# NickB42/mri-image-generation

Hardware: NVIDIA B200
Metric: volumes/sec (3D LDM DDPM sampling) (higher is better)
Workload: dtype bf16

## Files before the change

mri_image_generation_b200/csrc/gemm_tc.cu:

```cuda
#include <cuda.h>
#include <cuda_bf16.h>
#include <cuda_runtime.h>
#include <stdlib.h>
#include <string.h>

#include "../../include/mri_b200.h"
#include "common.h"
#include "ptx.cuh"

#ifdef MRI_GEMM_FINE_TRACE
#define FT_START() do { if (trace != nullptr) ft_t = clock64(); } while (0)
#define FT_ADD(k) do { if (trace != nullptr) { const long long n_ = clock64(); ft[k] += (unsigned long long)(n_ - ft_t); ft_t = n_; } } while (0)
#else
#define FT_START() do { } while (0)
#define FT_ADD(k) do { } while (0)
#endif

namespace mri {

constexpr int kBlockM = 128;
constexpr int kBlockK = 64;
constexpr int kUmmaK = 16;
constexpr int kSlabBytes = kBlockM * 128;
#ifndef MRI_EPI_WARPS
#define MRI_EPI_WARPS 4
#endif
constexpr int kEpiWarps = MRI_EPI_WARPS;
static_assert(kEpiWarps == 4 || kEpiWarps == 8, "one or two epilogue warps per TMEM lane quadrant");
constexpr int kSplit = kEpiWarps / 4;
constexpr int kEpiWarp0 = kEpiWarps == 8 ? 4 : 2;
constexpr int kThreads = (kEpiWarp0 + kEpiWarps) * 32;
constexpr int kEpiThreads = kEpiWarps * 32;
constexpr int kRegsProducer = 104, kRegsEpilogue = 200;
constexpr int kMaxStages = 8;
constexpr int kChunkBytes = kBlockM * 128;
constexpr int kStagingBytes = 2 * kChunkBytes;
constexpr int kPartialLd = 256;
constexpr int kMaxStatGroups = 32;
constexpr int kSmemLimit = 227 * 1024;
constexpr int kXTileBytes = 2 * 160 * 128;
constexpr int kXYTileBytes = 2 * 180 * 128;
constexpr int kXStages = 3;

__host__ __device__ inline int stage_bytes(int block_n, int swap_ab) {
  return swap_ab ? 3 * kSlabBytes : kSlabBytes + block_n * 128;
}

struct Work {
  int cls, n0, nbox;
  int tix[2][4], org[2][4];
};

struct Geom {
  int boxes_per_class;
  int groups_per_class;
  long long n_tiles;
  float rcp_ntn, rcp_gpc, rcp_te[4];
  int te[4], od[4];
};

__device__ __forceinline__ void fdivmod(int n, int d, float rcp, int& q, int& r) {
  q = __float2int_rz(__int2float_rn(n) * rcp);
  r = n - q * d;
  if (r < 0) {
    --q;
    r += d;
  } else if (r >= d) {
    ++q;
    r -= d;
  }
}

__device__ __forceinline__ Geom make_geom(const MriGemmArgs& p) {
  Geom g;
  g.boxes_per_class = p.tiles[0] * p.tiles[1] * p.tiles[2] * p.tiles[3];
  g.groups_per_class = p.swap_ab ? (g.boxes_per_class + 1) / 2 : g.boxes_per_class;
  g.n_tiles = (long long)p.n_tiles_n * p.n_class * g.groups_per_class;
  g.rcp_ntn = 1.0f / (float)p.n_tiles_n;
  g.rcp_gpc = 1.0f / (float)g.groups_per_class;
  const int f = p.tile_fast_dim;
#pragma unroll
  for (int k = 0; k < 4; ++k) {
    g.od[k] = (f == 0) ? k : (k == 0 ? f : (k <= f ? k - 1 : k));
    g.te[k] = g.od[k] == 0 ? p.tiles[0] : (g.od[k] == 1 ? p.tiles[1] : (g.od[k] == 2 ? p.tiles[2] : p.tiles[3]));
    g.rcp_te[k] = 1.0f / (float)g.te[k];
  }
  return g;
}

__device__ __forceinline__ int pick4(const int (&a)[4], int i) {
  return i == 0 ? a[0] : (i == 1 ? a[1] : (i == 2 ? a[2] : a[3]));
}

__device__ __forceinline__ void decode_tile(const MriGemmArgs& p, const Geom& g, int tile, Work& w) {
  int nt, pr;
  fdivmod(tile, p.n_tiles_n, g.rcp_ntn, pr, nt);
  int rem;
  fdivmod(pr, g.groups_per_class, g.rcp_gpc, w.cls, rem);
  w.n0 = nt * p.block_n;
  int b0 = rem;
  w.nbox = 1;
  if (p.swap_ab) {
    b0 = 2 * rem;
    w.nbox = (b0 + 1 < g.boxes_per_class) ? 2 : 1;
  }
#pragma unroll
  for (int h = 0; h < 2; ++h) {
    int b = b0 + h;
    int v[4];
#pragma unroll
    for (int k = 0; k < 4; ++k) {
      int qn;
      fdivmod(b, g.te[k], g.rcp_te[k], qn, v[k]);
      b = qn;
    }
#pragma unroll
    for (int i = 0; i < 4; ++i) {
      w.tix[h][i] = g.od[0] == i ? v[0] : (g.od[1] == i ? v[1] : (g.od[2] == i ? v[2] : v[3]));
      w.org[h][i] = w.tix[h][i] * p.box[i];
    }
  }
}

struct Sched {
  int n_kb, G, GA, q;
  long long rem_units;
  long long n_tiles, rem;
};

__device__ __forceinline__ Sched make_sched(const MriGemmArgs& p, long long n_tiles, int G) {
  Sched s;
  s.n_kb = p.n_kb;
  s.G = G;
  s.n_tiles = n_tiles;
  if (p.sched == 0) {
    s.q = 0;
    s.rem = 0;
    s.rem_units = 0;
    s.GA = 0;
  } else {
    s.q = (int)(n_tiles / G);
    s.rem = n_tiles - (long long)s.q * G;
    s.rem_units = s.rem * p.n_kb;
    const int min_share = (p.n_kb + 3) / 4 > 8 ? (p.n_kb + 3) / 4 : 8;
    const long long ga = s.rem_units / min_share;
    s.GA = (int)(ga < 1 ? (s.rem > 0 ? 1 : 0) : (ga > G ? G : ga));
  }
  return s;
}

__device__ __forceinline__ void range_a(const Sched& s, int r, long long& u0, long long& u1) {
  if (r >= s.GA) {
    u0 = u1 = s.rem_units;
    return;
  }
  u0 = s.rem_units * r / s.GA;
  u1 = s.rem_units * (r + 1) / s.GA;
}

struct SegIter {
  long long u, u1;
  long long tb, tb1;
  int n_kb;
  __device__ __forceinline__ void init(const MriGemmArgs& p, const Sched& s, int r) {
    n_kb = s.n_kb;
    if (p.sched == 0) {
      u = u1 = 0;
      tb = s.n_tiles * r / s.G;
      tb1 = s.n_tiles * (r + 1) / s.G;
    } else {
      range_a(s, r, u, u1);
      tb = s.rem + (long long)r * s.q;
      tb1 = tb + s.q;
    }
  }
  __device__ __forceinline__ bool next(int& tile, int& kb0, int& len, long long& seg_end) {
    if (u < u1) {
      tile = (int)(u / n_kb);
      kb0 = (int)(u - (long long)tile * n_kb);
      const long long left = u1 - u;
      len = (int)(left < (long long)(n_kb - kb0) ? left : (long long)(n_kb - kb0));
      u += len;
      seg_end = u;
      return true;
    }
    if (tb < tb1) {
      tile = (int)tb++;
      kb0 = 0;
      len = n_kb;
      seg_end = -1;
      return true;
    }
    return false;
  }
};

__device__ __forceinline__ uint32_t ld_acquire_gpu(const int32_t* p) {
  uint32_t v;
  asm volatile("ld.acquire.gpu.global.u32 %0, [%1];" : "=r"(v) : "l"(p) : "memory");
  return v;
}
__device__ __forceinline__ void st_release_gpu(int32_t* p, uint32_t v) {
  asm volatile("st.release.gpu.global.u32 [%0], %1;" ::"l"(p), "r"(v) : "memory");
}

__device__ __forceinline__ int count_contributors(const Sched& s, int my_r, long long pos,
                                                  long long tile_end) {
  int n = 0;
  int rr = my_r + 1;
  while (pos < tile_end) {
    long long a, b;
    range_a(s, rr, a, b);
    pos = b < tile_end ? b : tile_end;
    ++rr;
    ++n;
  }
  return n;
}

__device__ __forceinline__ void wait_contributors(const MriGemmArgs& p, int first_cta, int n) {
  for (int j = 0; j < n; ++j) {
    const int32_t* f = p.sk_flags + (first_cta - j);
    const uint64_t t0 = globaltimer_ns();
    while (ld_acquire_gpu(f) == 0u) {
      if (globaltimer_ns() - t0 > 4000000000ull) {
        printf("mri_b200: stream-K partial wait timeout (block %d waits for %d)\n",
               (int)blockIdx.x, first_cta - j);
        __trap();
      }
    }
  }
}

__device__ __forceinline__ float4* partial_ptr(const MriGemmArgs& p, int cta, int lane128, int col) {
  return reinterpret_cast<float4*>(p.sk_partials) +
         ((size_t)cta * (kPartialLd / 4) + (size_t)(col >> 2)) * kBlockM + lane128;
}

__global__ void __launch_bounds__(kThreads, 1)
gemm_tc_kernel(const __grid_constant__ MriGemmArgs p) {
  extern __shared__ uint8_t smem_raw[];
  __shared__ __align__(8) uint64_t bars[2 * kMaxStages + 5 + kXStages];
  __shared__ uint32_t tmem_holder;
  __shared__ double s_stats[kMaxStatGroups * 2];
  __shared__ int s_pos_info[kBlockM];
  __shared__ uint32_t s_vmask[4];
  __shared__ uint32_t s_winfo[kMaxStages];

  const int warp = uniform((int)(threadIdx.x >> 5));
  const int lane = threadIdx.x & 31;

  const uint32_t smem_base = (smem_u32(smem_raw) + 1023u) & ~1023u;
  const int S = p.stages;
  const int block_n = p.block_n;
  const bool swap = p.swap_ab != 0;
  const int sbytes = stage_bytes(block_n, p.swap_ab);
  const uint32_t stag = smem_base + (uint32_t)(p.xreuse ? S * kSlabBytes + (p.xreuse == 2 ? 2 * kXYTileBytes : ((p.staging2 || p.stages > 4) ? 2 : kXStages) * kXTileBytes)
                                                        : S * sbytes);
  const uint32_t bar0 = smem_u32(bars);
  auto full_bar = [&](int s) { return bar0 + 8u * s; };
  auto empty_bar = [&](int s) { return bar0 + 8u * (kMaxStages + s); };
  auto tmem_full_bar = [&](int b) { return bar0 + 8u * (2 * kMaxStages + b); };
  auto tmem_empty_bar = [&](int b) { return bar0 + 8u * (2 * kMaxStages + 2 + b); };
  const uint32_t resid_bar = bar0 + 8u * (2 * kMaxStages + 4);
  auto xempty_bar = [&](int s) { return bar0 + 8u * (2 * kMaxStages + 5 + s); };
  const bool xreuse = p.xreuse != 0;
  const bool xy = p.xreuse == 2;
  const int XS = (xy || p.staging2 || p.stages > 4) ? 2 : kXStages;
  const uint32_t x_tile_bytes = xy ? (uint32_t)kXYTileBytes : (uint32_t)kXTileBytes;
  const int x_box_rows = xy ? 180 : 160;
  const uint32_t x_ring = smem_base + (uint32_t)(S * kSlabBytes);

  const int n_kb = p.n_kb;
  const int G = (int)gridDim.x;
  const int my_r = G - 1 - (int)blockIdx.x;
  __shared__ Geom s_geom;
  __shared__ Sched s_sch;
  if (threadIdx.x == 0) {
    s_geom = make_geom(p);
    s_sch = make_sched(p, s_geom.n_tiles, G);
  }
  const Geom& geom = s_geom;
  const Sched& sch = s_sch;
  const int rows_in_box = p.box[0] * p.box[1] * p.box[2] * p.box[3];
  const bool dual = !swap && block_n <= 128;

  if (warp == 0 && lane == 0) {
    for (int s = 0; s < S; ++s) {
      mbar_init(full_bar(s), 1);
      mbar_init(empty_bar(s), 1);
    }
    for (int b = 0; b < 2; ++b) {
      mbar_init(tmem_full_bar(b), 1);
      mbar_init(tmem_empty_bar(b), kEpiThreads / 32);
    }
    mbar_init(resid_bar, 1);
    for (int xs = 0; xs < kXStages; ++xs) mbar_init(xempty_bar(xs), 1);
// ... 780 lines not shown
                      const float x = ((vm >> i) & 1u) ? f[i] : 0.f;
                      s_sum += x;
                      s_sq = fmaf(x, x, s_sq);
                    }
                  }
                }
#pragma unroll
                for (int i = 0; i < 16; ++i) {
                  const __nv_bfloat16 o = __float2bfloat16_rn(f[i]);
                  asm volatile("st.shared.u16 [%0], %1;" ::"r"(swz8[i & 7] + rowb + (uint32_t)i * 128u),
                               "h"(*reinterpret_cast<const uint16_t*>(&o))
                               : "memory");
                }
              }
            }
            FT_ADD(4);
            if (per_pos_sample) flush_pp(pp_sum, pp_sq, pp_sample);
            if (uniform_sample && !smem_stats) reduce_acc_stats();
            FT_ADD(5);
            fence_proxy_async_smem();
            FT_ADD(9);
            named_bar_sync(1, kEpiThreads);
            FT_ADD(6);
            if (epi_tid == 0) {
              tma_store_5d(o_map, sset, t.n0, oh[0], oh[1], oh[2], oh[3]);
              if (chunk1)
                tma_store_5d(o_map, sset + kChunkBytes, t.n0 + 64, oh[0], oh[1], oh[2], oh[3]);
              tma_store_commit();
            }
            FT_ADD(7);
          }
        }
        tc_fence_before();
        __syncwarp();
        if (lane == 0) mbar_arrive(tmem_empty_bar(buf));
        if (n_contrib > 0 && epi_tid == 0) {
          for (int j = 0; j < n_contrib; ++j) p.sk_flags[contrib_cta0 - j] = 0;
        }
      }
      ++seg;
      FT_ADD(8);
    }
#ifdef MRI_GEMM_FINE_TRACE
    if (trace != nullptr && (epi_tid == 0 || epi_tid == 96)) {
      uint64_t* row = p.trace + (size_t)((epi_tid == 0 ? 1 : 2) * gridDim.x + blockIdx.x) * 16;
      for (int k = 0; k < 12; ++k) row[k] = ft[k];
    }
#endif
    if (swap) reduce_acc_stats();
    if (smem_stats) flush_smem_stats();
    if (epi_tid == 0) tma_store_wait_all();
    if (trace != nullptr && epi_tid == 0) {
      trace[5] = (uint64_t)clock64();
      trace[6] = globaltimer_ns();
    }
  }

  tc_fence_before();
  __syncthreads();
  if (warp == 1) tmem_dealloc(tmem_base, 512);
}

}

using namespace mri;

static int pick_stages(int block_n, int swap_ab, int requested, int staging2 = 0) {
  const int budget = kSmemLimit - 1024 - kStagingBytes * (staging2 ? 2 : 1);
  int s = budget / stage_bytes(block_n, swap_ab);
  if (s > kMaxStages) s = kMaxStages;
  if (requested >= 2 && requested < s) s = requested;
  return s;
}

extern "C" int mri_gemm_smem_bytes(int block_n, int swap_ab, int stages) {
  return pick_stages(block_n, swap_ab, stages) * stage_bytes(block_n, swap_ab) + kStagingBytes + 1024;
}

static int usable_sms(int hw) {
  static const int env = [] {
    const char* e = getenv("MRI_GEMM_SMS");
    return e != nullptr ? atoi(e) : 0;
  }();
  return (env >= 8 && env < hw) ? env : hw;
}

extern "C" int mri_gemm_workspace_bytes(int* n_ctas_out) {
  int dev = 0, sms = 0;
  cudaError_t e = cudaGetDevice(&dev);
  if (e == cudaSuccess) e = cudaDeviceGetAttribute(&sms, cudaDevAttrMultiProcessorCount, dev);
  if (e != cudaSuccess) return set_cuda_error(e, "mri_gemm_workspace_bytes");
  sms = usable_sms(sms);
  if (n_ctas_out) *n_ctas_out = sms;
  const long long bytes = (long long)sms * kBlockM * kPartialLd * 4 + 1024;
  return (int)bytes;
}

extern "C" int mri_gemm_launch(const MriGemmArgs* a, void* stream) {
  if (a == nullptr) return set_error(-1, "mri_gemm_launch: null args");
  const int bn = a->block_n;
  if (!(bn == 16 || bn == 32 || bn == 64 || bn == 128 || bn == 256))
    return set_error(-2, "mri_gemm_launch: block_n must be 16/32/64/128/256");
  if (a->n_kb < 1 || a->n_class < 1) return set_error(-2, "mri_gemm_launch: empty K loop");
  long long rows = 1;
  long long boxes = 1;
  for (int i = 0; i < 4; ++i) {
    if (a->box[i] < 1 || a->tiles[i] < 1) return set_error(-2, "mri_gemm_launch: bad box/tiles");
    rows *= a->box[i];
    boxes *= a->tiles[i];
  }
  const int swap = a->swap_ab != 0;
  if (swap && (bn != 128 || a->n_total % 64 != 0 || a->out_f32 || a->bias_m != nullptr ||
               a->bz_sel[0] > 1 || a->bz_sel[1] > 1))
    return set_error(-2, "mri_gemm_launch: swap_ab needs block_n 128, n_total % 64 == 0, bf16 "
                         "output, no bias_m and class-only weight selection");
  if (a->r_base != nullptr) {
    bool ok = true;
    for (int i = 0; i < 4; ++i) ok = ok && (a->r_stride[i] % 8 == 0);
    for (int c = 0; c < a->n_class && c < 8; ++c) ok = ok && (a->r_cls_off[c] % 8 == 0);
    if (!ok) return set_error(-2, "mri_gemm_launch: residual strides/offsets must be multiples of 8");
  }
  const long long tiles = (long long)a->n_tiles_n * a->n_class * (swap ? (boxes + 1) / 2 : boxes);
  if (rows > kBlockM) return set_error(-2, "mri_gemm_launch: box has more than 128 rows");
  if (tiles >= (1LL << 24) || boxes + 1 >= (1LL << 24))
    return set_error(-2, "mri_gemm_launch: more than 2^24 tiles (tile decoding uses float reciprocals)");
  if (tiles > 0x7fffffffLL / a->n_kb) return set_error(-2, "mri_gemm_launch: too many work units");
  if (a->n_total % 8 != 0) return set_error(-2, "mri_gemm_launch: n_total must be a multiple of 8");
  if (a->stats != nullptr && !a->swap_ab && (a->stats_cpg < 8 || a->stats_cpg % 8 != 0))
    return set_error(-2, "mri_gemm_launch: statistics need channel groups in multiples of 8");
  if (a->stats != nullptr && a->stats_cpg < 1) return set_error(-2, "mri_gemm_launch: stats_cpg < 1");
  if (a->r_base != nullptr && a->out_f32)
    return set_error(-2, "mri_gemm_launch: residual input requires bf16 output");
  if (a->r_base != nullptr && a->n_class > 8)
    return set_error(-2, "mri_gemm_launch: residual supports at most 8 output classes");
  if ((a->r_base != nullptr) != (a->r_maps != nullptr))
    return set_error(-2, "mri_gemm_launch: residual needs both r_maps and r_base");
  if (a->out_f32 && bn > 128)
    return set_error(-2, "mri_gemm_launch: fp32 output needs block_n <= 128");
  static int n_sms = 0;
  if (n_sms == 0) {
    int dev = 0;
    cudaError_t e = cudaGetDevice(&dev);
    if (e == cudaSuccess) e = cudaDeviceGetAttribute(&n_sms, cudaDevAttrMultiProcessorCount, dev);
    if (e != cudaSuccess) return set_cuda_error(e, "cudaDeviceGetAttribute(SM count)");
    n_sms = usable_sms(n_sms);
  }
  MriGemmArgs k = *a;
  k.staging2 = (swap && a->n_kb <= 40) ? 1 : 0;
  k.stages = pick_stages(bn, swap, a->stages, k.staging2);
  int smem = k.stages * stage_bytes(bn, swap) + kStagingBytes * (k.staging2 ? 2 : 1) + 1024;
  if (a->tile_fast_dim < 0 || a->tile_fast_dim > 3) return set_error(-2, "mri_gemm_launch: tile_fast_dim must be 0..3");
  if (a->xreuse) {
    if (!swap || a->box[0] != 8 || rows != kBlockM || a->bz_sel[0] > 1 || a->bz_sel[1] > 1)
      return set_error(-2, "mri_gemm_launch: xreuse needs swap_ab and boxes of 8 x 16 positions");
    static const int env_xring = [] {
      const char* e = getenv("MRI_GEMM_XRING");
      return e != nullptr ? atoi(e) : 0;
    }();
    k.stages = (env_xring == 3 || k.staging2) ? 4 : 6;
    smem = k.stages * kSlabBytes + ((k.staging2 || k.stages > 4) ? 2 : kXStages) * kXTileBytes +
           kStagingBytes * (k.staging2 ? 2 : 1) + 1024;
    if (a->xreuse == 2) {
      if (a->box[1] != 16) return set_error(-2, "mri_gemm_launch: xreuse 2 needs boxes of 8 x 16 positions");
      k.stages = k.staging2 ? 4 : 6;
      smem = k.stages * kSlabBytes + 2 * kXYTileBytes + kStagingBytes * (k.staging2 ? 2 : 1) + 1024;
    }
  }
  long long grid = tiles < n_sms ? tiles : n_sms;
  if (k.sched != 0) {
    if (k.sk_partials == nullptr || k.sk_flags == nullptr)
      return set_error(-2, "mri_gemm_launch: stream-K schedule needs the workspace");
    if (tiles < n_sms) {
      const long long units = tiles * k.n_kb;
      const int min_share = (k.n_kb + 3) / 4 > 8 ? (k.n_kb + 3) / 4 : 8;
      const long long want = units / min_share > tiles ? units / min_share : tiles;
      grid = want < n_sms ? want : n_sms;
    }
    if (grid > k.sk_ctas) return set_error(-2, "mri_gemm_launch: stream-K workspace too small");
  }
  static int configured_smem = 0;
  if (smem > configured_smem) {
    cudaError_t e = cudaFuncSetAttribute(gemm_tc_kernel, cudaFuncAttributeMaxDynamicSharedMemorySize,
                                         smem);
    if (e != cudaSuccess) return set_cuda_error(e, "cudaFuncSetAttribute(gemm_tc_kernel)");
    configured_smem = smem;
  }
  gemm_tc_kernel<<<(unsigned)grid, kThreads, smem, (cudaStream_t)stream>>>(k);
  return check_launch("gemm_tc_kernel");
}

typedef CUresult (*EncodeTiledFn)(CUtensorMap*, CUtensorMapDataType, cuuint32_t, void*,
                                  const cuuint64_t*, const cuuint64_t*, const cuuint32_t*,
                                  const cuuint32_t*, CUtensorMapInterleave, CUtensorMapSwizzle,
                                  CUtensorMapL2promotion, CUtensorMapFloatOOBfill);

extern "C" int mri_tmap_encode(void* out_map_host, uint64_t global_addr, int dtype, int rank,
                               const uint64_t* dims, const uint64_t* strides_bytes,
                               const uint32_t* box, int swizzle) {
  static EncodeTiledFn fn = nullptr;
  if (fn == nullptr) {
    void* sym = nullptr;
    cudaDriverEntryPointQueryResult qres;
    cudaError_t e = cudaGetDriverEntryPoint("cuTensorMapEncodeTiled", &sym, cudaEnableDefault, &qres);
    if (e != cudaSuccess || sym == nullptr || qres != cudaDriverEntryPointSuccess)
      return set_error(-3, "mri_tmap_encode: cuTensorMapEncodeTiled not available (no driver?)");
    fn = reinterpret_cast<EncodeTiledFn>(sym);
  }
  if (rank < 1 || rank > 5) return set_error(-2, "mri_tmap_encode: rank must be 1..5");
  cuuint64_t gdim[5], gstr[4];
  cuuint32_t bx[5], es[5];
  for (int i = 0; i < rank; ++i) {
    gdim[i] = dims[i];
    bx[i] = box[i];
    es[i] = 1;
    if (i + 1 < rank) gstr[i] = strides_bytes[i];
  }
  const CUtensorMapDataType dt =
      dtype == 0 ? CU_TENSOR_MAP_DATA_TYPE_BFLOAT16 : CU_TENSOR_MAP_DATA_TYPE_FLOAT32;
  const CUtensorMapSwizzle sw = swizzle == 3   ? CU_TENSOR_MAP_SWIZZLE_128B
                                : swizzle == 2 ? CU_TENSOR_MAP_SWIZZLE_64B
                                : swizzle == 1 ? CU_TENSOR_MAP_SWIZZLE_32B
                                               : CU_TENSOR_MAP_SWIZZLE_NONE;
  alignas(64) CUtensorMap tmp;
  CUresult r = fn(&tmp, dt, (cuuint32_t)rank, reinterpret_cast<void*>(global_addr), gdim, gstr, bx,
                  es, CU_TENSOR_MAP_INTERLEAVE_NONE, sw, CU_TENSOR_MAP_L2_PROMOTION_L2_256B,
                  CU_TENSOR_MAP_FLOAT_OOB_FILL_NONE);
  if (r != CUDA_SUCCESS) {
    char msg[256];
    snprintf(msg, sizeof msg,
             "cuTensorMapEncodeTiled failed (CUresult %d): rank %d dims [%llu %llu %llu %llu %llu] "
             "box [%u %u %u %u %u]",
             (int)r, rank, (unsigned long long)gdim[0], (unsigned long long)(rank > 1 ? gdim[1] : 0),
             (unsigned long long)(rank > 2 ? gdim[2] : 0), (unsigned long long)(rank > 3 ? gdim[3] : 0),
             (unsigned long long)(rank > 4 ? gdim[4] : 0), bx[0], rank > 1 ? bx[1] : 0,
             rank > 2 ? bx[2] : 0, rank > 3 ? bx[3] : 0, rank > 4 ? bx[4] : 0);
    return set_error(-4, msg);
  }
  memcpy(out_map_host, &tmp, sizeof(CUtensorMap));
  return 0;
}
```

mri_image_generation_b200/plan.py:

```python
from __future__ import annotations

import ctypes as C
import itertools
import os
from dataclasses import dataclass, field
from typing import List, Optional, Sequence, Tuple

import numpy as np
import torch

from . import _lib

BLOCK_M = 128
BLOCK_K = 64


def _esize(dt: torch.dtype) -> int:
    return {torch.bfloat16: 2, torch.float32: 4}[dt]


@dataclass
class TView:
    base: torch.Tensor
    dims: Tuple[int, ...]
    strides: Tuple[int, ...]
    offset: int = 0

    def __post_init__(self):
        assert len(self.dims) == len(self.strides) and self.strides[0] == 1
        assert self.base.is_contiguous()

    @property
    def esize(self) -> int:
        return _esize(self.base.dtype)

    def ptr(self) -> int:
        return self.base.data_ptr() + self.offset * self.esize


@dataclass
class MapSpec:
    view: TView
    box: Tuple[int, ...]
    swizzle: int


def pad_rank(view: TView, box: Sequence[int], rank: int) -> Tuple[TView, Tuple[int, ...]]:
    dims, strides, box = list(view.dims), list(view.strides), list(box)
    while len(dims) < rank:
        big = max(d * s for d, s in zip(dims, strides))
        big = (big + 7) // 8 * 8
        dims.append(1)
        strides.append(big)
        box.append(1)
    return TView(view.base, tuple(dims), tuple(strides), view.offset), tuple(box)


def encode_maps(specs: Sequence[MapSpec], device) -> torch.Tensor:
    lib = _lib.load()
    host = np.zeros((len(specs), 128), dtype=np.uint8)
    for i, sp in enumerate(specs):
        v = sp.view
        rank = len(v.dims)
        es = v.esize
        dims = (C.c_uint64 * rank)(*v.dims)
        strides = (C.c_uint64 * max(rank - 1, 1))(*[s * es for s in v.strides[1:]] or [0])
        box = (C.c_uint32 * rank)(*sp.box)
        buf = (C.c_uint8 * 128)()
        rc = lib.mri_tmap_encode(C.addressof(buf), v.ptr(), 0 if v.base.dtype == torch.bfloat16 else 1,
                                 rank, dims, strides, box, sp.swizzle)
        _lib.check(rc, "mri_tmap_encode")
        host[i] = np.frombuffer(buf, dtype=np.uint8)
    return torch.from_numpy(host).to(device)


class _Workspace:

    def __init__(self, device):
        n = C.c_int(0)
        nbytes = _lib.load().mri_gemm_workspace_bytes(C.byref(n))
        if nbytes <= 0:
            _lib.check(nbytes, "mri_gemm_workspace_bytes")
        self.n_ctas = n.value
        self.buf = torch.zeros(nbytes, dtype=torch.uint8, device=device)
        self.partials_ptr = self.buf.data_ptr()
        self.flags_ptr = self.buf.data_ptr() + nbytes - 1024


_WORKSPACES = {}


def gemm_workspace(device) -> _Workspace:
    dev = torch.device(device)
    idx = dev.index if dev.index is not None else torch.cuda.current_device()
    ws = _WORKSPACES.get(idx)
    if ws is None:
        with torch.cuda.device(idx):
            ws = _Workspace(torch.device("cuda", idx))
        _WORKSPACES[idx] = ws
    return ws


def choose_box(ext: Sequence[int], prefer_unit: Sequence[int] = ()) -> Tuple[int, int, int, int]:
    ext = list(ext) + [1] * (4 - len(ext))

    def cands(e):
        c = {d for d in range(1, min(e, BLOCK_M) + 1) if e % d == 0}
        c |= {p for p in (1, 2, 4, 8, 16, 32, 64, 128) if p <= e}
        c.add(min(e, BLOCK_M))
        return sorted(c)

    best, best_key = None, None
    total = ext[0] * ext[1] * ext[2] * ext[3]
    for b in itertools.product(*[cands(e) for e in ext]):
        rows = b[0] * b[1] * b[2] * b[3]
        if rows > BLOCK_M:
            continue
        tiles = 1
        for e, bb in zip(ext, b):
            tiles *= -(-e // bb)
        eff = total / (tiles * BLOCK_M)
        unit_pen = sum(1 for i in prefer_unit if b[i] != 1)
        score = eff
        for i in prefer_unit:
            if b[i] != 1 and (rows // b[i]) % 16 != 0:
                score = eff * 0.75
        key = (round(score, 6), -unit_pen, b[0] == 8, b[0], b[1], b[2])
        if best_key is None or key > best_key:
            best, best_key = b, key
    return best


@dataclass
class GemmPlan:
    a_maps: List[MapSpec]
    b_map: Optional[MapSpec]
    o_maps: List[MapSpec]
    ktable: np.ndarray
    tiles: Tuple[int, int, int, int]
    box: Tuple[int, int, int, int]
    ext: Tuple[int, int, int, int]
    block_n: int
    n_total: int
    r_maps: Optional[List[MapSpec]] = None
    bz_sel: Tuple[int, int] = (0, 0)
    sample_dim: int = 0
    out_f32: bool = False
    bias: Optional[torch.Tensor] = None
    bias_m: Optional[torch.Tensor] = None
    rowbias: Optional[torch.Tensor] = None
    rowbias_ld: int = 0
    stats: Optional[torch.Tensor] = None
    stats_ld: int = 0
    stats_cpg: int = 0
    stages: int = 0
    sched: Optional[int] = None
    swap_ab: Optional[bool] = None
    tile_fast_dim: int = 0
    xreuse: int = 0
    a_maps_std: Optional[List[MapSpec]] = None
    trace: Optional[torch.Tensor] = None
    name: str = ""
    flops: int = 0
    _args: Optional[_lib.MriGemmArgs] = field(default=None, repr=False)
    _keep: list = field(default_factory=list, repr=False)

    @property
    def n_class(self) -> int:
        return self.ktable.shape[0]

    @property
    def n_kb(self) -> int:
        return self.ktable.shape[1]

    @property
    def n_tiles_n(self) -> int:
        return -(-self.n_total // self.block_n)

    def pick_swap(self) -> bool:
        if self.swap_ab is not None:
            return self.swap_ab
        env = os.environ.get("MRI_GEMM_SWAP")
        if env:
            return bool(int(env)) and self.block_n == 128 and self.n_total % 64 == 0
        return (self.block_n == 128 and self.n_total % 64 == 0 and not self.out_f32
                and self.bias_m is None and max(self.bz_sel) <= 1)

    def grid(self) -> int:
        t = self.tiles
        boxes = t[0] * t[1] * t[2] * t[3]
        groups = -(-boxes // 2) if self.pick_swap() else boxes
        return groups * self.n_tiles_n * self.n_class

    def pick_stages(self) -> int:
        if self.stages:
            return self.stages
        env = os.environ.get("MRI_GEMM_STAGES")
        return int(env) if env else 0

    def pick_sched(self, n_sms: int) -> int:
        if self.sched is not None:
            return self.sched
        env = os.environ.get("MRI_GEMM_SCHED")
        if env:
            return int(env)
        tiles = self.grid()
        if self.n_kb < 8:
            return 0
        waves = tiles / n_sms
        return 1 if -(-tiles // n_sms) / waves > 1.02 else 0

    def materialize(self, device) -> None:
        maps = list(self.a_maps) + [self.b_map] + list(self.o_maps) + list(self.r_maps or [])
        blob = encode_maps(maps, device)
        na, no = len(self.a_maps), len(self.o_maps)
        base = blob.data_ptr()
        kt = torch.from_numpy(np.ascontiguousarray(self.ktable, dtype=np.int32)).to(device)
        self._keep = [blob, kt]
        a = _lib.MriGemmArgs()
        a.a_maps = base
        a.b_map = base + 128 * na
        a.o_maps = base + 128 * (na + 1)
        if self.r_maps:
            if len(self.r_maps) > 8:
                raise _lib.MriError("residual input supports at most 8 output classes")
            v0 = self.r_maps[0].view
            assert v0.base.dtype == torch.bfloat16
            a.r_maps = base + 128 * (na + 1 + no)
            a.r_base = v0.base.data_ptr()
            for ci, m in enumerate(self.r_maps):
                assert m.view.base is v0.base and m.view.strides == v0.strides
                a.r_cls_off[ci] = m.view.offset
            for i in range(4):
                a.r_stride[i] = v0.strides[1 + i]
        else:
            a.r_maps = None
            a.r_base = None
        a.ktable = kt.data_ptr()
        a.n_kb, a.n_class = self.n_kb, self.n_class
        for i in range(4):
            a.tiles[i], a.box[i], a.ext[i] = self.tiles[i], self.box[i], self.ext[i]
        a.n_tiles_n, a.block_n, a.n_total = self.n_tiles_n, self.block_n, self.n_total
        a.bz_sel[0], a.bz_sel[1] = self.bz_sel
        a.sample_dim = self.sample_dim
        a.out_f32 = 1 if self.out_f32 else 0
        a.bias = self.bias.data_ptr() if self.bias is not None else None
        a.bias_m = self.bias_m.data_ptr() if self.bias_m is not None else None
        a.rowbias = self.rowbias.data_ptr() if self.rowbias is not None else None
        a.rowbias_ld = self.rowbias_ld
        a.stats = self.stats.data_ptr() if self.stats is not None else None
        a.stats_ld, a.stats_cpg = self.stats_ld, self.stats_cpg
        a.stages = self.pick_stages()
        ws = gemm_workspace(device)
        a.sk_partials, a.sk_flags, a.sk_ctas = ws.partials_ptr, ws.flags_ptr, ws.n_ctas
        a.sched = self.pick_sched(ws.n_ctas)
        a.swap_ab = 1 if self.pick_swap() else 0
        a.xreuse = int(self.xreuse)
        a.tile_fast_dim = int(self.tile_fast_dim)
        if self.xreuse and not a.swap_ab:
            raise _lib.MriError("xreuse plans need the swap_ab tile shape")
        a.trace = self.trace.data_ptr() if self.trace is not None else None
        self._args = a

    def launch(self, stream: Optional[int] = None) -> None:
        if self._args is None:
            raise _lib.MriError("GemmPlan.launch before materialize()")
        rc = _lib.load().mri_gemm_launch(C.byref(self._args),
                                         stream if stream is not None else _lib.current_stream_ptr())
        _lib.check(rc, f"mri_gemm_launch[{self.name}]")

    def simulate(self) -> None:
        nt_n = self.n_tiles_n
        rows_in_box = int(np.prod(self.box))
        for cls in range(self.n_class):
            for tix in itertools.product(*[range(t) for t in reversed(self.tiles)]):
                tix = tuple(reversed(tix))
                org = [tix[i] * self.box[i] for i in range(4)]
                rl = _row_coords(self.box)
                valid = torch.ones(rows_in_box, dtype=torch.bool)
                for i in range(4):
                    valid &= (org[i] + rl[i]) < self.ext[i]
                sample = (org[self.sample_dim - 1] + rl[self.sample_dim - 1]) if self.sample_dim else \
                    torch.zeros(rows_in_box, dtype=torch.long)
                for nt in range(nt_n):
                    n0 = nt * self.block_n
                    acc = torch.zeros(rows_in_box, self.block_n, dtype=torch.float32)
                    sel = lambda s: 0 if s == 0 else (cls if s == 1 else tix[s - 2])
                    bz = (sel(self.bz_sel[0]), sel(self.bz_sel[1]))
                    for kb in range(self.n_kb):
                        e = self.ktable[cls, kb]
                        am = self.a_maps[int(e[0])]
                        coords = [int(e[1])] + [org[i] + int(e[2 + i]) for i in range(4)]
                        a = _load_box(am.view, coords, (BLOCK_K,) + tuple(self.box)).reshape(rows_in_box, BLOCK_K)
                        b = _load_box(self.b_map.view, [int(e[6]), n0, bz[0], bz[1]],
                                      self.b_map.box).reshape(self.block_n, BLOCK_K)
                        acc += a @ b.t()
                    ncols = torch.arange(n0, n0 + self.block_n)
                    colok = ncols < self.n_total
                    if self.bias is not None:
                        acc += torch.where(colok, self.bias[ncols.clamp(max=self.bias.numel() - 1)],
                                           torch.zeros(()))[None, :]
                    if self.bias_m is not None:
                        x1 = (org[0] + rl[0]).clamp(max=self.bias_m.numel() - 1)
                        acc += torch.where(valid, self.bias_m[x1], torch.zeros(()))[:, None]
                    if self.rowbias is not None:
                        if self.rowbias_ld == 0:
                            rb = self.rowbias.reshape(1, -1)
                        else:
                            rb = self.rowbias.reshape(-1, self.rowbias_ld) if self.rowbias.dim() == 1 \
                                else self.rowbias
                        smp = sample.clamp(max=rb.shape[0] - 1)
                        add = rb[smp][:, ncols.clamp(max=rb.shape[1] - 1)]
                        acc += torch.where(valid[:, None] & colok[None, :], add, torch.zeros(()))
                    om = self.o_maps[cls]
                    ocoords = [n0] + org
                    if self.r_maps is not None:
                        rm = self.r_maps[cls]
                        res = _load_box(rm.view, ocoords, _full_box(rm, self.block_n))
                        acc += res.reshape(rows_in_box, self.block_n)
                    if self.stats is not None:
                        for g0 in range(0, self.block_n, self.stats_cpg):
                            if n0 + g0 >= self.n_total:
                                break
                            blk = acc[:, g0:g0 + self.stats_cpg]
                            g = (n0 + g0) // self.stats_cpg
                            for smp in torch.unique(sample[valid]).tolist():
                                m = valid & (sample == smp)
                                self.stats[smp, g, 0] += blk[m].sum()
                                self.stats[smp, g, 1] += (blk[m] ** 2).sum()
                    _store_box(om.view, ocoords, _full_box(om, self.block_n),
                               acc.reshape(*reversed(self.box), self.block_n), self.n_total)


def _full_box(m: MapSpec, block_n: int) -> Tuple[int, ...]:
    return (block_n,) + tuple(m.box[1:])


def _row_coords(box):
    r = torch.arange(int(np.prod(box)))
    out = []
    for b in box:
        out.append(r % b)
        r = r // b
    return out


def _box_index(view: TView, coords, box):
    rank = len(view.dims)
    idx = None
    mask = None
    shape_tail = []
    for i in range(rank):
        ar = coords[i] + torch.arange(box[i])
        ok = (ar >= 0) & (ar < view.dims[i])
        shp = [1] * rank
        shp[rank - 1 - i] = box[i]
        term = (ar.clamp(0, view.dims[i] - 1) * view.strides[i]).reshape(shp)
        okr = ok.reshape(shp)
        idx = term if idx is None else idx + term
        mask = okr if mask is None else mask & okr
    return idx + view.offset, mask


def _load_box(view: TView, coords, box) -> torch.Tensor:
    idx, mask = _box_index(view, coords, box)
    flat = view.base.reshape(-1)
    vals = flat[idx.reshape(-1)].float().reshape(idx.shape)
    return torch.where(mask, vals, torch.zeros(()))


def _store_box(view: TView, coords, box, vals: torch.Tensor, n_total: int) -> None:
    idx, mask = _box_index(view, coords, box)
    flat = view.base.reshape(-1)
    sel = mask.reshape(-1)
    flat[idx.reshape(-1)[sel]] = vals.reshape(-1)[sel].to(flat.dtype)



def _act_view(x: torch.Tensor, ndim: int) -> TView:
    shp = list(x.shape)
    C_ = shp[-1]
    sp = shp[1:-1]
    assert len(sp) == ndim
    dims, strides = [C_], [1]
    s = C_
    for e in reversed(sp):
        dims.append(e)
        strides.append(s)
        s *= e
    dims.append(shp[0])
    strides.append(s)
    v = TView(x, tuple(dims), tuple(strides))
    v, _ = pad_rank(v, [1] * len(dims), 5)
    return v


def _parity_view(x: torch.Tensor, ndim: int, par: Sequence[int]) -> TView:
    shp = list(x.shape)
    C_ = shp[-1]
    sp = shp[1:-1]
    dims, strides = [C_], [1]
    s = C_
    off = 0
    for i, e in enumerate(reversed(sp)):
        assert e % 2 == 0, "stride-2 paths need even spatial sizes"
        dims.append(e // 2)
        strides.append(2 * s)
        off += par[i] * s
        s *= e
    dims.append(shp[0])
    strides.append(s)
    v = TView(x, tuple(dims), tuple(strides), off)
    v, _ = pad_rank(v, [1] * len(dims), 5)
    return v


def _out_swizzle(chunk_bytes: int) -> int:
    return 3 if chunk_bytes == 128 else 0


def _out_chunk(block_n: int, out_f32: bool) -> int:
    full = 32 if out_f32 else 64
    return min(block_n, full)


def pick_block_n(cout_pad: int) -> int:
    if cout_pad % 64 == 0:
        return 128
    for bn in (32, 16):
        if cout_pad % bn == 0:
            return bn
    raise ValueError(f"Cout {cout_pad} must be a multiple of 16")


@dataclass
class ConvSource:
    x: torch.Tensor
    taps: bool = True


def _spatial_ext(y: torch.Tensor, ndim: int):
    sp = list(y.shape[1:-1])
    ext = list(reversed(sp)) + [y.shape[0]]
    sample_dim = ndim + 1
    while len(ext) < 4:
        ext.append(1)
    return tuple(ext), sample_dim


def conv_plan(sources: Sequence[ConvSource], wmat: torch.Tensor, y: torch.Tensor, ksize: int,
              *, bias=None, rowbias=None, rowbias_ld=0, residual: Optional[torch.Tensor] = None,
              stats=None, stats_cpg=0, block_n: Optional[int] = None, stages=0, name="",
              xreuse=None, out_f32: bool = False) -> GemmPlan:
    assert y.dtype == (torch.float32 if out_f32 else torch.bfloat16)
    assert not (out_f32 and residual is not None)
    ndim = y.dim() - 2
    ext, sample_dim = _spatial_ext(y, ndim)
    box = choose_box(ext, prefer_unit=(sample_dim - 1,))
    cout_pad = y.shape[-1]
    bn = block_n or pick_block_n(cout_pad)
    p = ksize // 2
    env_x = os.environ.get("MRI_GEMM_XREUSE")
    if xreuse is None:
        level = int(env_x) if env_x in ("0", "1", "2") else 1
    elif isinstance(xreuse, bool):
        level = 1 if xreuse else 0
    else:
        level = int(xreuse)
    use_x = bool(level >= 1 and ksize == 3 and bn == 128 and cout_pad % 64 == 0 and box[0] == 8
                 and int(np.prod(box)) == BLOCK_M and os.environ.get("MRI_GEMM_SWAP", "1") != "0"
                 and not out_f32)
    use_xy = bool(use_x and level >= 2 and box[1] == 16)
    a_maps, a_std, rows = [], [], []
    bk = 0
    for si, src in enumerate(sources):
        Ci = src.x.shape[-1]
        assert Ci % BLOCK_K == 0, f"source channels {Ci} must be a multiple of 64"
        assert list(src.x.shape[:-1]) == list(y.shape[:-1])
        a_std.append(MapSpec(_act_view(src.x, ndim), (BLOCK_K,) + box, 3))
        xbox = (BLOCK_K, 10, 18) + tuple(box[2:]) if use_xy else (BLOCK_K, 10) + tuple(box[1:])
        a_maps.append(MapSpec(_act_view(src.x, ndim), xbox, 3) if use_x else a_std[-1])
        if not src.taps:
            for c0 in range(0, Ci, BLOCK_K):
                rows.append([si, c0, 0, 0, 0, 0, bk, 1])
                bk += BLOCK_K
        elif use_xy:
            for ot in itertools.product(range(ksize), repeat=ndim - 2):
                for c0 in range(0, Ci, BLOCK_K):
                    for kh in range(ksize):
                        for kw in range(ksize):
                            tap = tuple(ot) + (kh, kw)
                            tap_index = 0
                            for t_ in tap:
                                tap_index = tap_index * ksize + t_
                            offs = [k - p for k in reversed(tap)] + [0] * (4 - ndim)
                            rows.append([si, c0] + offs + [bk + tap_index * Ci + c0,
                                                           1 if (kh == 0 and kw == 0) else 0])
            bk += (ksize ** ndim) * Ci
        elif use_x:
            for ot in itertools.product(range(ksize), repeat=ndim - 1):
                for c0 in range(0, Ci, BLOCK_K):
                    for kw in range(ksize):
                        tap = tuple(ot) + (kw,)
                        tap_index = 0
                        for t_ in tap:
                            tap_index = tap_index * ksize + t_
                        offs = [k - p for k in reversed(tap)] + [0] * (4 - ndim)
                        rows.append([si, c0] + offs + [bk + tap_index * Ci + c0, 1 if kw == 0 else 0])
            bk += (ksize ** ndim) * Ci
        else:
            for tap in itertools.product(range(ksize), repeat=ndim):
                offs = [k - p for k in reversed(tap)] + [0] * (4 - ndim)
                for c0 in range(0, Ci, BLOCK_K):
                    rows.append([si, c0] + offs + [bk, 0])
                    bk += BLOCK_K
    assert wmat.shape == (cout_pad, bk), (wmat.shape, cout_pad, bk)
    kt = np.asarray(rows, dtype=np.int32)[None]
    bview = TView(wmat, (bk, cout_pad, 1, 1), (1, bk, _rup8(bk * cout_pad), _rup8(bk * cout_pad)))
    chunk = _out_chunk(bn, out_f32)
    omap = MapSpec(_act_view(y, ndim), (chunk,) + box, _out_swizzle(chunk * (4 if out_f32 else 2)))
    rmaps = None
    if residual is not None:
        assert residual.shape == y.shape
        rmaps = [MapSpec(_act_view(residual, ndim), (chunk,) + box, _out_swizzle(chunk * 2))]
    tiles = tuple(-(-e // b) for e, b in zip(ext, box))
    m_rows = int(np.prod(ext))
    return GemmPlan(a_maps=a_maps, b_map=MapSpec(bview, (BLOCK_K, bn, 1, 1), 3), o_maps=[omap],
                    r_maps=rmaps, ktable=kt, tiles=tiles, box=box, ext=ext, block_n=bn, out_f32=out_f32,
                    n_total=cout_pad, sample_dim=sample_dim, bias=bias, rowbias=rowbias,
                    rowbias_ld=rowbias_ld, stats=stats, stats_ld=(stats.shape[1] if stats is not None else 0),
                    stats_cpg=stats_cpg, stages=stages, name=name, flops=2 * m_rows * cout_pad * bk,
                    xreuse=(2 if use_xy else 1) if use_x else 0, a_maps_std=a_std if use_x else None,
                    tile_fast_dim=_depth_first(ndim, ksize, tiles))


def _depth_first(ndim: int, ksize: int, tiles) -> int:
    env = os.environ.get("MRI_GEMM_TILE_ORDER")
    if env is not None:
        return int(env)
    return 2 if (ndim == 3 and ksize > 1 and tiles[2] > 1) else 0


def _rup8(n: int) -> int:
    return (n + 7) // 8 * 8


def down_conv_plan(x: torch.Tensor, wmat: torch.Tensor, y: torch.Tensor, *, bias=None, stats=None,
                   stats_cpg=0, block_n=None, stages=0, name="",
                   residual: Optional[torch.Tensor] = None, out_f32: bool = False) -> GemmPlan:
    ndim = y.dim() - 2
    ext, sample_dim = _spatial_ext(y, ndim)
    box = choose_box(ext, prefer_unit=(sample_dim - 1,))
    Ci, cout_pad = x.shape[-1], y.shape[-1]
    assert Ci % BLOCK_K == 0
    bn = block_n or pick_block_n(cout_pad)
    PA = [(1, -1), (0, 0), (1, 0), (0, 1)]
    pars = list(itertools.product((0, 1), repeat=ndim))
    a_maps = [MapSpec(_parity_view(x, ndim, par), (BLOCK_K,) + box, 3) for par in pars]
    par_index = {par: i for i, par in enumerate(pars)}
    rows, bk = [], 0
    for tap in itertools.product(range(4), repeat=ndim):
        kk = list(reversed(tap))
        par = tuple(PA[k][0] for k in kk)
        offs = [PA[k][1] for k in kk] + [0] * (4 - ndim)
        for c0 in range(0, Ci, BLOCK_K):
            rows.append([par_index[par], c0] + offs + [bk, 0])
            bk += BLOCK_K
    assert wmat.shape == (cout_pad, bk)
    kt = np.asarray(rows, dtype=np.int32)[None]
    bview = TView(wmat, (bk, cout_pad, 1, 1), (1, bk, _rup8(bk * cout_pad), _rup8(bk * cout_pad)))
    assert y.dtype == (torch.float32 if out_f32 else torch.bfloat16) and not (out_f32 and residual is not None)
    chunk = _out_chunk(bn, out_f32)
    omap = MapSpec(_act_view(y, ndim), (chunk,) + box, _out_swizzle(chunk * (4 if out_f32 else 2)))
    tiles = tuple(-(-e // b) for e, b in zip(ext, box))
    rmaps = None
    if residual is not None:
        assert residual.shape == y.shape
        rmaps = [MapSpec(_act_view(residual, ndim), (chunk,) + box, _out_swizzle(chunk * 2))]
    return GemmPlan(a_maps=a_maps, b_map=MapSpec(bview, (BLOCK_K, bn, 1, 1), 3), o_maps=[omap], out_f32=out_f32,
                    r_maps=rmaps, ktable=kt, tiles=tiles, box=box, ext=ext, block_n=bn, n_total=cout_pad,
                    sample_dim=sample_dim, bias=bias, stats=stats,
                    stats_ld=(stats.shape[1] if stats is not None else 0), stats_cpg=stats_cpg,
                    stages=stages, name=name, flops=2 * int(np.prod(ext)) * cout_pad * bk)


_CT_TAPS = {0: [(1, 0), (3, -1)], 1: [(0, 1), (2, 0)]}


def up_conv_plan(x: torch.Tensor, wmat: torch.Tensor, y: torch.Tensor, *, bias=None, stats=None,
                 stats_cpg=0, block_n=None, stages=0, name="",
                 residual: Optional[torch.Tensor] = None, out_f32: bool = False) -> GemmPlan:
    ndim = y.dim() - 2
    in_ext, sample_dim = _spatial_ext(x, ndim)
    box = choose_box(in_ext, prefer_unit=(sample_dim - 1,))
    Ci, cout_pad = x.shape[-1], y.shape[-1]
    assert Ci % BLOCK_K == 0
    for a, b in zip(x.shape[1:-1], y.shape[1:-1]):
        assert b == 2 * a
    bn = block_n or pick_block_n(cout_pad)
    classes = list(itertools.product((0, 1), repeat=ndim))
    a_maps = [MapSpec(_act_view(x, ndim), (BLOCK_K,) + box, 3)]
    kts = []
    K = (2 ** ndim) * Ci
    for rho in classes:
        rows, bk = [], 0
        for combo in itertools.product((0, 1), repeat=ndim):
            offs = [_CT_TAPS[rho[i]][combo[i]][1] for i in range(ndim)] + [0] * (4 - ndim)
            for c0 in range(0, Ci, BLOCK_K):
                rows.append([0, c0] + offs + [bk, 0])
                bk += BLOCK_K
        assert bk == K
        kts.append(rows)
    kt = np.asarray(kts, dtype=np.int32)
    ncls = len(classes)
    assert wmat.shape == (ncls, cout_pad, K), (wmat.shape, (ncls, cout_pad, K))
    bview = TView(wmat, (K, cout_pad, ncls, 1), (1, K, K * cout_pad, _rup8(K * cout_pad * ncls)))
    assert y.dtype == (torch.float32 if out_f32 else torch.bfloat16) and not (out_f32 and residual is not None)
    chunk = _out_chunk(bn, out_f32)
    o_maps = [MapSpec(_parity_view(y, ndim, rho), (chunk,) + box, _out_swizzle(chunk * (4 if out_f32 else 2)))
              for rho in classes]
    tiles = tuple(-(-e // b) for e, b in zip(in_ext, box))
    rmaps = None
    if residual is not None:
        assert residual.shape == y.shape
        rmaps = [MapSpec(_parity_view(residual, ndim, rho), (chunk,) + box, _out_swizzle(chunk * 2))
                 for rho in classes]
    return GemmPlan(a_maps=a_maps, b_map=MapSpec(bview, (BLOCK_K, bn, 1, 1), 3), o_maps=o_maps, out_f32=out_f32,
                    r_maps=rmaps, ktable=kt, tiles=tiles, box=box, ext=in_ext, block_n=bn, n_total=cout_pad,
                    bz_sel=(1, 0), sample_dim=sample_dim, bias=bias, stats=stats,
                    stats_ld=(stats.shape[1] if stats is not None else 0), stats_cpg=stats_cpg,
                    stages=stages, name=name, flops=2 * int(np.prod(in_ext)) * cout_pad * K * ncls)


def matrix_plan(a: TView, a_box_rows: Tuple[int, int, int, int], b: TView, o: TView, *, K: int,
                n_total: int, block_n: int, ext, tiles, bz_sel=(0, 0), sample_dim=0, out_f32=False,
                bias=None, bias_m=None, stats=None, stats_cpg=0, stages=0, name="",
                flops=0) -> GemmPlan:
    n_kb = -(-K // BLOCK_K)
    kt = np.zeros((1, n_kb, 8), dtype=np.int32)
    kt[0, :, 1] = np.arange(n_kb) * BLOCK_K
    kt[0, :, 6] = np.arange(n_kb) * BLOCK_K
    chunk = _out_chunk(block_n, out_f32)
    es = 4 if out_f32 else 2
    return GemmPlan(a_maps=[MapSpec(a, (BLOCK_K,) + tuple(a_box_rows), 3)],
                    b_map=MapSpec(b, (BLOCK_K, block_n, 1, 1), 3),
                    o_maps=[MapSpec(o, (chunk,) + tuple(a_box_rows), _out_swizzle(chunk * es))],
                    ktable=kt, tiles=tuple(tiles), box=tuple(a_box_rows), ext=tuple(ext),
                    block_n=block_n, n_total=n_total, bz_sel=bz_sel, sample_dim=sample_dim,
                    out_f32=out_f32, bias=bias, bias_m=bias_m, stats=stats,
                    stats_ld=(stats.shape[1] if stats is not None else 0), stats_cpg=stats_cpg,
                    stages=stages, name=name, flops=flops)


def pick_wgrad_splits(base: int, total_mt: int, sms: int = 148, max_waves: int = 4) -> int:
    best, best_cost = 1, None
    for waves in range(1, max_waves + 1):
        splits = min(total_mt, (waves * sms) // base)
        if splits < 1:
            continue
        w_real = -(-(base * splits) // sms)
        cost = w_real * -(-total_mt // splits)
        if best_cost is None or cost < best_cost * 0.97:
            best, best_cost = splits, cost
    if best_cost is None:
        return 1
    return best


@dataclass
class WgradPlan:
    fwd: GemmPlan
    dy: torch.Tensor
    dw: torch.Tensor
    n_total: int
    group: int = 4
    stages: int = 2
    splits: int = 0
    name: str = ""
    dy_views: Optional[List[TView]] = None
    _args: Optional[_lib.MriWgradArgs] = field(default=None, repr=False)
    _launches: list = field(default_factory=list, repr=False)
    _keep: list = field(default_factory=list, repr=False)

    def dy_specs(self) -> List[MapSpec]:
        if self.dy_views is not None:
            return [MapSpec(v, (BLOCK_K,) + tuple(self.fwd.box), 3) for v in self.dy_views]
        out = []
        for om in self.fwd.o_maps:
            v = om.view
            assert v.base.shape == self.dy.shape and v.base.dtype == torch.bfloat16
            out.append(MapSpec(TView(self.dy, v.dims, v.strides, v.offset),
                               (BLOCK_K,) + tuple(self.fwd.box), 3))
        return out
# ... 177 lines not shown
```

Before: 0.8793.

## Extend x-reuse conv path to any axis with box 8; add wide stream-K schedule

The conv plan now permutes the spatial axes so that whichever axis has a box extent of 8 becomes the fast x-reuse axis. This lets 3D convolutions whose tile box is not 8 along x1 still use the halo-reusing A-tile path, with the tap table, output and residual maps and depth ordering remapped to match. Separately, a new stream-K mode (sched=2) uses a finer minimum share per CTA. The planner picks it when the default split would leave the busiest CTA noticeably overloaded for deep-K GEMMs. The axis permutation adds complexity to the TMA views and to the tap ordering, and getting either wrong would produce incorrect results.

```diff
diff --git a/mri_image_generation_b200/csrc/gemm_tc.cu b/mri_image_generation_b200/csrc/gemm_tc.cu
--- a/mri_image_generation_b200/csrc/gemm_tc.cu
+++ b/mri_image_generation_b200/csrc/gemm_tc.cu
@@ -122,6 +122,9 @@
   }
 }
 
+#ifndef MRI_SK_WIDE_DIV
+#define MRI_SK_WIDE_DIV 8
+#endif
 struct Sched {
   int n_kb, G, GA, q;
   long long rem_units;
@@ -142,7 +145,8 @@
     s.q = (int)(n_tiles / G);
     s.rem = n_tiles - (long long)s.q * G;
     s.rem_units = s.rem * p.n_kb;
-    const int min_share = (p.n_kb + 3) / 4 > 8 ? (p.n_kb + 3) / 4 : 8;
+    const int div = p.sched == 2 ? MRI_SK_WIDE_DIV : 4;
+    const int min_share = (p.n_kb + div - 1) / div > 8 ? (p.n_kb + div - 1) / div : 8;
     const long long ga = s.rem_units / min_share;
     s.GA = (int)(ga < 1 ? (s.rem > 0 ? 1 : 0) : (ga > G ? G : ga));
   }
@@ -1229,7 +1233,7 @@
   if (a->tile_fast_dim < 0 || a->tile_fast_dim > 3) return set_error(-2, "mri_gemm_launch: tile_fast_dim must be 0..3");
   if (a->xreuse) {
     if (!swap || a->box[0] != 8 || rows != kBlockM || a->bz_sel[0] > 1 || a->bz_sel[1] > 1)
-      return set_error(-2, "mri_gemm_launch: xreuse needs swap_ab and boxes of 8 x 16 positions");
+      return set_error(-2, "mri_gemm_launch: xreuse needs swap_ab and boxes of 128 positions, 8 along x1");
     static const int env_xring = [] {
       const char* e = getenv("MRI_GEMM_XRING");
       return e != nullptr ? atoi(e) : 0;
@@ -1244,6 +1248,7 @@
     }
   }
   long long grid = tiles < n_sms ? tiles : n_sms;
+  if (k.sched < 0 || k.sched > 2) return set_error(-2, "mri_gemm_launch: sched must be 0, 1 or 2");
   if (k.sched != 0) {
     if (k.sk_partials == nullptr || k.sk_flags == nullptr)
       return set_error(-2, "mri_gemm_launch: stream-K schedule needs the workspace");
diff --git a/mri_image_generation_b200/plan.py b/mri_image_generation_b200/plan.py
--- a/mri_image_generation_b200/plan.py
+++ b/mri_image_generation_b200/plan.py
@@ -85,6 +85,32 @@
         self.buf = torch.zeros(nbytes, dtype=torch.uint8, device=device)
         self.partials_ptr = self.buf.data_ptr()
         self.flags_ptr = self.buf.data_ptr() + nbytes - 1024
+
+
+def stream_k_segments(n_tiles: int, n_kb: int, n_sms: int, sched: int) -> List[List[Tuple[int, int, int]]]:
+    G = min(n_tiles, n_sms)
+    min_share = max((n_kb + 3) // 4, 8)
+    if sched != 0 and n_tiles < n_sms:
+        G = min(max(n_tiles * n_kb // min_share, n_tiles), n_sms)
+    if sched == 0:
+        return [[(t, 0, n_kb) for t in range(n_tiles * r // G, n_tiles * (r + 1) // G)] for r in range(G)]
+    q, rem = divmod(n_tiles, G)
+    units = rem * n_kb
+    share = max((n_kb + 7) // 8, 8) if sched == 2 else min_share
+    ga = units // share
+    GA = (1 if rem > 0 else 0) if ga < 1 else min(ga, G)
+    out = []
+    for r in range(G):
+        u, u1 = (units * r // GA, units * (r + 1) // GA) if r < GA else (units, units)
+        segs = []
+        while u < u1:
+            tile, kb0 = divmod(u, n_kb)
+            n = min(u1 - u, n_kb - kb0)
+            segs.append((tile, kb0, n))
+            u += n
+        segs += [(t, 0, n_kb) for t in range(rem + r * q, rem + (r + 1) * q)]
+        out.append(segs)
+    return out
 
 
 _WORKSPACES = {}
@@ -208,7 +234,13 @@
         if self.n_kb < 8:
             return 0
         waves = tiles / n_sms
-        return 1 if -(-tiles // n_sms) / waves > 1.02 else 0
+        if -(-tiles // n_sms) / waves <= 1.02:
+            return 0
+        if tiles >= n_sms and self.n_kb > 40:
+            busiest = max(sum(s[2] for s in r) for r in stream_k_segments(tiles, self.n_kb, n_sms, 1))
+            if busiest / (tiles * self.n_kb / n_sms) > 1.03:
+                return 2
+        return 1
 
     def materialize(self, device) -> None:
         maps = list(self.a_maps) + [self.b_map] + list(self.o_maps) + list(self.r_maps or [])
@@ -467,19 +499,27 @@
         level = 1 if xreuse else 0
     else:
         level = int(xreuse)
-    use_x = bool(level >= 1 and ksize == 3 and bn == 128 and cout_pad % 64 == 0 and box[0] == 8
+    axis = 0
+    if box[0] != 8 and ndim == 3:
+        axis = next((d for d in range(1, ndim) if box[d] == 8), 0)
+    use_x = bool(level >= 1 and ksize == 3 and bn == 128 and cout_pad % 64 == 0 and box[axis] == 8
                  and int(np.prod(box)) == BLOCK_M and os.environ.get("MRI_GEMM_SWAP", "1") != "0"
                  and not out_f32)
-    use_xy = bool(use_x and level >= 2 and box[1] == 16)
+    order = [axis] + [d for d in range(4) if d != axis] if use_x else [0, 1, 2, 3]
+    box, ext = tuple(box[d] for d in order), tuple(ext[d] for d in order)
+    sample_dim = order.index(sample_dim - 1) + 1
+    view = lambda x: _permute_view(_act_view(x, ndim), order)
+    use_xy = bool(use_x and level >= 2 and box[1] == 16 and axis == 0)
+    tap_axis = ndim - 1 - axis
     a_maps, a_std, rows = [], [], []
     bk = 0
     for si, src in enumerate(sources):
         Ci = src.x.shape[-1]
         assert Ci % BLOCK_K == 0, f"source channels {Ci} must be a multiple of 64"
         assert list(src.x.shape[:-1]) == list(y.shape[:-1])
-        a_std.append(MapSpec(_act_view(src.x, ndim), (BLOCK_K,) + box, 3))
+        a_std.append(MapSpec(view(src.x), (BLOCK_K,) + box, 3))
         xbox = (BLOCK_K, 10, 18) + tuple(box[2:]) if use_xy else (BLOCK_K, 10) + tuple(box[1:])
-        a_maps.append(MapSpec(_act_view(src.x, ndim), xbox, 3) if use_x else a_std[-1])
+        a_maps.append(MapSpec(view(src.x), xbox, 3) if use_x else a_std[-1])
         if not src.taps:
             for c0 in range(0, Ci, BLOCK_K):
                 rows.append([si, c0, 0, 0, 0, 0, bk, 1])
@@ -500,13 +540,14 @@
         elif use_x:
             for ot in itertools.product(range(ksize), repeat=ndim - 1):
                 for c0 in range(0, Ci, BLOCK_K):
-                    for kw in range(ksize):
-                        tap = tuple(ot) + (kw,)
+                    for kx in range(ksize):
+                        tap = tuple(ot[:tap_axis]) + (kx,) + tuple(ot[tap_axis:])
                         tap_index = 0
                         for t_ in tap:
                             tap_index = tap_index * ksize + t_
                         offs = [k - p for k in reversed(tap)] + [0] * (4 - ndim)
-                        rows.append([si, c0] + offs + [bk + tap_index * Ci + c0, 1 if kw == 0 else 0])
+                        offs = [offs[d] for d in order]
+                        rows.append([si, c0] + offs + [bk + tap_index * Ci + c0, 1 if kx == 0 else 0])
             bk += (ksize ** ndim) * Ci
         else:
             for tap in itertools.product(range(ksize), repeat=ndim):
@@ -518,11 +559,11 @@
     kt = np.asarray(rows, dtype=np.int32)[None]
     bview = TView(wmat, (bk, cout_pad, 1, 1), (1, bk, _rup8(bk * cout_pad), _rup8(bk * cout_pad)))
     chunk = _out_chunk(bn, out_f32)
-    omap = MapSpec(_act_view(y, ndim), (chunk,) + box, _out_swizzle(chunk * (4 if out_f32 else 2)))
+    omap = MapSpec(view(y), (chunk,) + box, _out_swizzle(chunk * (4 if out_f32 else 2)))
     rmaps = None
     if residual is not None:
         assert residual.shape == y.shape
-        rmaps = [MapSpec(_act_view(residual, ndim), (chunk,) + box, _out_swizzle(chunk * 2))]
+        rmaps = [MapSpec(view(residual), (chunk,) + box, _out_swizzle(chunk * 2))]
     tiles = tuple(-(-e // b) for e, b in zip(ext, box))
     m_rows = int(np.prod(ext))
     return GemmPlan(a_maps=a_maps, b_map=MapSpec(bview, (BLOCK_K, bn, 1, 1), 3), o_maps=[omap],
@@ -531,14 +572,20 @@
                     rowbias_ld=rowbias_ld, stats=stats, stats_ld=(stats.shape[1] if stats is not None else 0),
                     stats_cpg=stats_cpg, stages=stages, name=name, flops=2 * m_rows * cout_pad * bk,
                     xreuse=(2 if use_xy else 1) if use_x else 0, a_maps_std=a_std if use_x else None,
-                    tile_fast_dim=_depth_first(ndim, ksize, tiles))
-
-
-def _depth_first(ndim: int, ksize: int, tiles) -> int:
+                    tile_fast_dim=_depth_first(ndim, ksize, tiles, order.index(2)))
+
+
+def _permute_view(v: TView, order: Sequence[int]) -> TView:
+    dims = (v.dims[0],) + tuple(v.dims[1 + d] for d in order)
+    strides = (1,) + tuple(v.strides[1 + d] for d in order)
+    return TView(v.base, dims, strides, v.offset)
+
+
+def _depth_first(ndim: int, ksize: int, tiles, depth: int = 2) -> int:
     env = os.environ.get("MRI_GEMM_TILE_ORDER")
     if env is not None:
         return int(env)
-    return 2 if (ndim == 3 and ksize > 1 and tiles[2] > 1) else 0
+    return depth if (ndim == 3 and ksize > 1 and tiles[depth] > 1) else 0
 
 
 def _rup8(n: int) -> int:
```

Result: faster. 0.8993, median of 6 (+2.3%).
